# victorramirez952/tomography_3d_reconstructor

Hardware: AMD Instinct MI355X
Metric: Mvoxels/s (SDF+MC) on 1024^3 ellipsoid stack; achieved HBM GB/s vs peak (higher is better)
Workload: dtype f64

## Files before the change

### include/tomo_hip.h

```cpp
#ifndef TOMO_HIP_H
#define TOMO_HIP_H

#include <stddef.h>
#include <stdint.h>

#ifdef __cplusplus
extern "C" {
#endif

#define TOMO_OK 0
#define TOMO_E_ARG (-1)
#define TOMO_E_LAUNCH (-2)
#define TOMO_E_SIZE (-3)
#define TOMO_E_WORKSPACE (-4)

int tomo_abi_version(void);
const char *tomo_error_string(int code);
int tomo_host_mc_cell(const float *h_v, double iso, int8_t *h_tris, int *h_uses_centre);
double tomo_host_mc_edge_offset(double va, double vb);
void tomo_host_mc_centre_offset(const double *h_v8, double *h_out3);

int tomo_host_checksum(const void *h_data, int64_t nbytes, int nthreads, uint64_t *h_out);
int tomo_host_checksum_impl(const void *h_data, int64_t nbytes, int nthreads, int impl, uint64_t *h_out);
int64_t tomo_host_checksum_chunk_bytes(void);
// ... 196 lines not shown
                   const double *xt, double r2, int level, int32_t *map, void *workspace, int64_t workspace_bytes, void *stream);
int tomo_edt_threshold_masked(const uint64_t *sites, int nz, int ny, int nx, const double *zt, const double *yt, const double *xt,
                              int inside, double r2, int keep_less, const uint64_t *mask, uint64_t *out, void *workspace,
                              int64_t workspace_bytes, void *stream);
int tomo_edt_thickness_finish(int32_t *map, const uint64_t *bits, int nz, int ny, int nx, const float *values, int levels,
                              int64_t *counts, void *stream);
int tomo_pack_threshold(const uint8_t *grey, uint64_t *bits, int nz, int ny, int nx, int threshold, void *stream);
int tomo_obj_write(const char *path, const void *vertices, int vertex_is_double, int64_t nv, const int64_t *faces,
                   int64_t nf, int nthreads);
int tomo_obj_block_format(int kind, const void *h_rows, int64_t n, int nthreads, void **h_block, int64_t *h_nbytes);
int tomo_obj_block_pwrite(const char *path, int64_t offset, const void *h_block);
void tomo_obj_block_free(void *h_block);

int tomo_extend_bits(const uint64_t *bits, uint64_t *ext, int nz, int ny, int nx, int pad, void *stream);
int tomo_field_fill(const uint64_t *ext, float *field, int nz, int ny, int nx, int pad, int gaussian,
                    unsigned long long *signs, uint8_t *gcls, void *stream);
int tomo_field_fill_bits(const uint64_t *bits, float *field, int nz, int ny, int nx, int pad, unsigned long long *signs,
                         uint8_t *gcls, void *stream);
int64_t tomo_field_span_bytes(int nz, int ny, int nx, int pad);
int tomo_field_fill_bits_sparse(const uint64_t *bits, float *field, int nz, int ny, int nx, int pad, unsigned long long *signs,
                                uint8_t *gcls, uint8_t *span_ws, void *stream);
int64_t tomo_sign_rows(int Ny);
int64_t tomo_sign_buffer_words(int Nz, int Ny, int Nx, int xorg);
int tomo_field_signs(const float *field, int Nz, int Ny, int Nx, int64_t pitch, int xorg, double iso, int z_begin,
                     int z_end, unsigned long long *signs, uint8_t *gcls, void *stream);

int tomo_mc_classify(const unsigned long long *signs, const uint8_t *gcls, int Nz, int Ny, int Nx, int xorg,
                     unsigned long long *seg_act, uint32_t *seg_cnt, void *stream);
int tomo_mc_scan_segments(const uint32_t *seg_cnt, int64_t nseg, uint32_t *seg_aoff, unsigned long long *totals,
                          void *workspace, int64_t workspace_bytes, void *stream);
int64_t tomo_mc_scan_workspace_bytes(int64_t n);
int tomo_mc_scan(const uint32_t *counts, int64_t n, uint32_t *off_a, uint32_t *off_b,
                 unsigned long long *totals, void *workspace, int64_t workspace_bytes, void *stream);
int tomo_mc_list(int Nz, int Ny, int Nx, int xorg, const uint32_t *seg_aoff, const unsigned long long *seg_act,
                 unsigned long long *vox_key, void *stream);
int tomo_mc_eval(const float *field, int Nz, int Ny, int Nx, int64_t pitch, int xorg, double iso,
                 const unsigned long long *vox_key, int64_t na, uint32_t *vox_counts, uint8_t *vox_flags, void *stream);
int tomo_mc_list_capped(int Nz, int Ny, int Nx, int xorg, const uint32_t *seg_aoff, const unsigned long long *seg_act,
                        unsigned long long *vox_key, int64_t cap, void *stream);
int tomo_mc_eval_capped(const float *field, int Nz, int Ny, int Nx, int64_t pitch, int xorg, double iso,
                        const unsigned long long *vox_key, int64_t cap, const unsigned long long *na_dev,
                        uint32_t *vox_counts, uint8_t *vox_flags, void *stream);
int tomo_mc_emit(const float *field, int Nz, int Ny, int Nx, int64_t pitch, int xorg, double iso,
                 const unsigned long long *vox_key, int64_t na, const unsigned long long *seg_act,
                 const uint32_t *seg_aoff, const uint32_t *vox_voff, const uint32_t *vox_foff, const uint8_t *vox_flags,
                 int z_offset, unsigned long long *vkey, float *vpos, int32_t *faces, unsigned long long *totals,
                 void *stream);

int tomo_mc_first_touch(const float *field, int Nz, int Ny, int Nx, int64_t pitch, int xorg, double iso,
                        const unsigned long long *vox_key, int64_t na, const unsigned long long *seg_act,
                        const uint32_t *seg_aoff, const uint32_t *vox_voff, const uint8_t *vox_flags, int mode,
                        uint32_t *created, const uint32_t *base, int32_t *ft_rank, unsigned long long *totals, void *stream);

int tomo_mc3_list(int Nz, int Ny, int Nx, int xorg, const uint32_t *seg_cnt, const unsigned long long *seg_act,
                  uint32_t *seg_blk, uint32_t *seg_aoff, unsigned long long *vox_key, int64_t cap, unsigned long long *tot,
                  void *stream);
int tomo_mc3_eval(const float *field, int Nz, int Ny, int Nx, int64_t pitch, int xorg, double iso,
                  const unsigned long long *vox_key, int64_t cap, const unsigned long long *tot, int z_offset,
                  uint32_t *vox_loc, int32_t *vox_til, uint8_t *vox_flags, uint16_t *vox_used, float *vox_f3, float *vox_c3,
                  uint32_t *blk3, void *stream);
int64_t tomo_mc3_slice_table_words(int Nz, int Ny);
int64_t tomo_mc3_sort_segments(int Nz, int Ny);
int tomo_mc3_scan(int Nz, int Ny, int Nx, int xorg, const uint32_t *seg_aoff, const uint32_t *vox_loc, int64_t cap,
                  uint32_t *blk3, uint32_t *slice_tab, unsigned long long *tot, int64_t cap_v, int64_t cap_f, void *stream);
int tomo_mc3_vertices(int Nz, int Ny, int Nx, int xorg, const unsigned long long *vox_key, int64_t cap,
                      const unsigned long long *tot, const uint32_t *vox_loc, const uint8_t *vox_flags, const float *vox_f3,
                      const float *vox_c3, const uint32_t *blk3, const uint32_t *slice_tab, int z_offset, int shift,
                      const double *cum, int64_t ncum, const double *adj, int64_t nadj, float mm_y, float mm_x, float *vrec,
                      uint32_t *keys, uint32_t *idx, void *stream);
int64_t tomo_mc3_sort_workspace_bytes(int64_t cap_v, int64_t nseg);
int tomo_mc3_sort_rank_top(const float *vrec, uint32_t *keys, uint32_t *idx, int64_t cap_v, int Nz, int Ny, const uint32_t *slice_tab,
                           unsigned long long *tot, float *uniq, int32_t *table, void *workspace, int64_t workspace_bytes,
                           float z_top, void *stream);
int tomo_mc3_sort_rank_fused(const float *vrec, const uint32_t *keys, int64_t cap_v, int Nz, int Ny, uint32_t *slice_tab,
                             unsigned long long *tot, float *uniq, int32_t *table, float z_top, void *stream);
int tomo_mc3_faces(int Nz, int Ny, int Nx, int xorg, const unsigned long long *vox_key, int64_t cap, unsigned long long *tot,
                   const unsigned long long *seg_act, const uint32_t *seg_aoff, const uint32_t *vox_loc, const int32_t *vox_til,
                   const uint16_t *vox_used, const uint32_t *blk3, const int32_t *table, int64_t *faces, int64_t cap_f,
                   void *stream);

int tomo_vertex_finalize(float *vpos, int64_t nv, int shift, const double *cum, int64_t ncum,
                         const double *adj, int64_t nadj, float mm_y, float mm_x, void *stream);
int64_t tomo_mesh_unique_workspace_bytes(int64_t nv);
int tomo_mesh_unique(const float *vpos, int64_t nv, float *uniq, int32_t *rank, unsigned long long *totals,
                     void *workspace, int64_t workspace_bytes, void *stream);
int tomo_mesh_lookup(const float *uniq, int64_t nu, const float *query, int64_t nq, int32_t *out,
                     unsigned long long *missing, void *stream);
int tomo_slab_top_rows(const float *uniq, const unsigned long long *tot, int64_t cap_v, int64_t cap, float *msg, void *stream);
int tomo_slab_lookup_summary(const float *uniq, const unsigned long long *tot, int64_t cap_v, const float *msg, int64_t cap,
                             int32_t *out, int64_t cap_top, int64_t caller_flags, unsigned long long *scratch, int64_t *summary,
                             void *stream);
int tomo_mc3_faces_slab(int Nz, int Ny, int Nx, int xorg, const unsigned long long *vox_key, int64_t cap, unsigned long long *tot,
                        const unsigned long long *seg_act, const uint32_t *seg_aoff, const uint32_t *vox_loc, const int32_t *vox_til,
                        const uint16_t *vox_used, const uint32_t *blk3, const int32_t *table, int64_t *faces, int64_t cap_f,
                        const int64_t *gathered, int rank, int world, const int32_t *ids_next, int64_t cap_top, int64_t cap_v,
                        void *stream);
int tomo_mesh_volume_area(const float *verts, const int64_t *faces, int64_t nf, double *out, void *stream);

int tomo_layer_colors(const void *verts, int is_f64, int64_t nv, int64_t stride, double start1, double end1, int enable1,
                      double start2, double end2, int enable2, uint8_t *rgba, void *stream);
int64_t tomo_mesh_edge_table_bytes(int64_t nf);
int tomo_mesh_edges(const int64_t *faces, int64_t nf, int64_t nv, void *table, int64_t table_bytes, unsigned long long *counters,
                    void *stream);
int tomo_mesh_seam_edges(const void *table, int64_t table_bytes, int64_t nf, int64_t first_ghost, unsigned long long *msg,
                         int64_t cap, unsigned long long *count, void *stream);
int tomo_mesh_seam_merge(const void *table, int64_t table_bytes, int64_t nf, const unsigned long long *msg, int64_t n,
// ... 21 lines not shown
```

### tomography_3d_reconstructor_amd/_lib.py

```python
import ctypes
import os
import subprocess

_HERE = os.path.dirname(os.path.abspath(__file__))
SO_PATH = os.environ.get("TOMO_LIB") or os.path.join(_HERE, "libtomo_hip.so")
CSRC = os.path.join(_HERE, "csrc")

_c_i = ctypes.c_int
_c_i64 = ctypes.c_int64
_c_p = ctypes.c_void_p
_c_d = ctypes.c_double
_c_f = ctypes.c_float

SIGNATURES = {
    "tomo_abi_version": (_c_i, []),
    "tomo_error_string": (ctypes.c_char_p, [_c_i]),
    "tomo_host_mc_cell": (_c_i, [_c_p, _c_d, _c_p, _c_p]),
    "tomo_host_mc_edge_offset": (_c_d, [_c_d, _c_d]),
    "tomo_host_mc_centre_offset": (None, [_c_p, _c_p]),
    "tomo_host_checksum": (_c_i, [_c_p, _c_i64, _c_i, _c_p]),
    "tomo_host_checksum_impl": (_c_i, [_c_p, _c_i64, _c_i, _c_i, _c_p]),
    "tomo_host_checksum_chunk_bytes": (_c_i64, []),
    "tomo_host_checksum_part": (_c_i, [_c_p, _c_i64, _c_i64, _c_i, _c_i, _c_p]),
    "tomo_host_checksum_fold": (_c_i, [_c_p, _c_i64, _c_i64, _c_p]),
# ... 87 lines not shown
    "tomo_thin_nodes": (_c_i, [_c_p, _c_i, _c_i, _c_i, _c_p, _c_p, _c_p, _c_p]),
    "tomo_thin_count": (_c_i, [_c_p, _c_i, _c_i, _c_i, _c_p, _c_i64, _c_p, _c_p, _c_p, _c_p, _c_p, _c_p, _c_p, _c_i, _c_i, _c_i64, _c_i64,
                               _c_p]),
    "tomo_branch_split": (_c_i, [_c_p, _c_i, _c_i, _c_i, _c_p, _c_p, _c_p, _c_p]),
    "tomo_branch_hist": (_c_i, [_c_p, _c_i, _c_i, _c_i, _c_p, _c_i64, _c_p, _c_p, _c_p, _c_p, _c_i64, _c_p, _c_p, _c_p, _c_i64, _c_p,
                                _c_p]),
    "tomo_branch_attach": (_c_i, [_c_p, _c_i, _c_i, _c_i, _c_p, _c_i64, _c_p, _c_p, _c_p, _c_p, _c_p, _c_p, _c_p, _c_p, _c_i64, _c_i64,
                                  _c_p]),
    "tomo_branch_lookup": (_c_i, [_c_p, _c_i, _c_i, _c_i, _c_p, _c_i64, _c_p, _c_p, _c_p, _c_i64, _c_p, _c_i64, _c_p, _c_p]),
    "tomo_branch_clear": (_c_i, [_c_p, _c_i, _c_i, _c_i, _c_p, _c_i64, _c_p, _c_p, _c_p, _c_p, _c_i64, _c_p, _c_p, _c_p]),
    "tomo_contact_count": (_c_i, [_c_p, _c_p, _c_i, _c_i, _c_i, _c_p, _c_p]),
    "tomo_contact_insert": (_c_i, [_c_p, _c_p, _c_i, _c_i, _c_i, _c_p, _c_p, _c_p, _c_p, _c_i64, _c_p, _c_p, _c_p, _c_p, _c_p, _c_p, _c_p,
                                   _c_p, _c_p]),
    "tomo_contact_hist": (_c_i, [_c_p, _c_p, _c_i, _c_i, _c_i, _c_p, _c_i64, _c_p, _c_p, _c_p, _c_p, _c_p, _c_i64, _c_p, _c_i64, _c_p, _c_p,
                                 _c_p]),
    "tomo_contact_finish": (_c_i, [_c_i64, _c_p, _c_i64, _c_p, _c_p, _c_p, _c_p, _c_p, _c_p, _c_p, _c_p, _c_p, _c_p, _c_i64, _c_p, _c_i, _c_i,
                                   _c_p, _c_p, _c_p]),
    "tomo_pack_threshold": (_c_i, [_c_p, _c_p, _c_i, _c_i, _c_i, _c_i, _c_p]),
    "tomo_obj_write": (_c_i, [ctypes.c_char_p, _c_p, _c_i, _c_i64, _c_p, _c_i64, _c_i]),
    "tomo_obj_block_format": (_c_i, [_c_i, _c_p, _c_i64, _c_i, ctypes.POINTER(_c_p), ctypes.POINTER(_c_i64)]),
    "tomo_obj_block_pwrite": (_c_i, [ctypes.c_char_p, _c_i64, _c_p]),
    "tomo_obj_block_free": (None, [_c_p]),
    "tomo_fill_holes_slice": (_c_i, [_c_p, _c_i, _c_i, _c_i, _c_i, _c_p, _c_p]),
    "tomo_fill_holes_ends": (_c_i, [_c_p, _c_i, _c_i, _c_i, _c_p, _c_p]),
    "tomo_pack_close_ends": (_c_i, [_c_p, _c_p, _c_i, _c_i, _c_i, _c_p, _c_p]),
    "tomo_pack_bits_pair": (_c_i, [_c_p, _c_p, _c_i, _c_p, _c_p, _c_i, _c_i, _c_i, _c_p]),
    "tomo_slab_edges": (_c_i, [_c_p, _c_p, _c_i, _c_i, _c_i, _c_i, _c_p, _c_p, _c_i, _c_i, _c_p, _c_p, _c_p, _c_i, _c_p, _c_p, _c_p, _c_p,
                               _c_i, _c_p, _c_p]),
    "tomo_pack_close_range": (_c_i, [_c_p, _c_p, _c_i, _c_i, _c_i, _c_i, _c_i, _c_p, _c_p, _c_i, _c_i, _c_p]),
    "tomo_close_ends_workspace_words": (_c_i64, [_c_i, _c_i, _c_i]),
    "tomo_close_ends_scan": (_c_i, [_c_p, _c_i, _c_i, _c_i, _c_p, _c_p]),
    "tomo_morph_fused": (_c_i, [_c_p, _c_p, _c_i, _c_i, _c_i, ctypes.c_uint32, _c_i, _c_p]),
    "tomo_smooth": (_c_i, [_c_p, _c_p, _c_i, _c_i, _c_i, _c_i, _c_i, _c_p]),
    "tomo_extend_bits": (_c_i, [_c_p, _c_p, _c_i, _c_i, _c_i, _c_i, _c_p]),
    "tomo_field_fill": (_c_i, [_c_p, _c_p, _c_i, _c_i, _c_i, _c_i, _c_i, _c_p, _c_p, _c_p]),
    "tomo_field_fill_bits": (_c_i, [_c_p, _c_p, _c_i, _c_i, _c_i, _c_i, _c_p, _c_p, _c_p]),
    "tomo_field_span_bytes": (_c_i64, [_c_i, _c_i, _c_i, _c_i]),
    "tomo_field_fill_bits_sparse": (_c_i, [_c_p, _c_p, _c_i, _c_i, _c_i, _c_i, _c_p, _c_p, _c_p, _c_p]),
    "tomo_sign_rows": (_c_i64, [_c_i]),
    "tomo_sign_buffer_words": (_c_i64, [_c_i, _c_i, _c_i, _c_i]),
    "tomo_field_signs": (_c_i, [_c_p, _c_i, _c_i, _c_i, _c_i64, _c_i, _c_d, _c_i, _c_i, _c_p, _c_p, _c_p]),
    "tomo_mc_classify": (_c_i, [_c_p, _c_p, _c_i, _c_i, _c_i, _c_i, _c_p, _c_p, _c_p]),
    "tomo_mc_scan_segments": (_c_i, [_c_p, _c_i64, _c_p, _c_p, _c_p, _c_i64, _c_p]),
    "tomo_mc_scan_workspace_bytes": (_c_i64, [_c_i64]),
    "tomo_mc_scan": (_c_i, [_c_p, _c_i64, _c_p, _c_p, _c_p, _c_p, _c_i64, _c_p]),
    "tomo_mc_list": (_c_i, [_c_i, _c_i, _c_i, _c_i, _c_p, _c_p, _c_p, _c_p]),
    "tomo_mc_eval": (_c_i, [_c_p, _c_i, _c_i, _c_i, _c_i64, _c_i, _c_d, _c_p, _c_i64, _c_p, _c_p, _c_p]),
    "tomo_mc_list_capped": (_c_i, [_c_i, _c_i, _c_i, _c_i, _c_p, _c_p, _c_p, _c_i64, _c_p]),
    "tomo_mc_eval_capped": (_c_i, [_c_p, _c_i, _c_i, _c_i, _c_i64, _c_i, _c_d, _c_p, _c_i64, _c_p, _c_p, _c_p, _c_p]),
    "tomo_mc_emit": (_c_i, [_c_p, _c_i, _c_i, _c_i, _c_i64, _c_i, _c_d, _c_p, _c_i64, _c_p, _c_p, _c_p, _c_p, _c_p, _c_i, _c_p,
                            _c_p, _c_p, _c_p, _c_p]),
    "tomo_mc_first_touch": (_c_i, [_c_p, _c_i, _c_i, _c_i, _c_i64, _c_i, _c_d, _c_p, _c_i64, _c_p, _c_p, _c_p, _c_p, _c_i, _c_p,
                                   _c_p, _c_p, _c_p, _c_p]),
    "tomo_mc3_list": (_c_i, [_c_i, _c_i, _c_i, _c_i, _c_p, _c_p, _c_p, _c_p, _c_p, _c_i64, _c_p, _c_p]),
    "tomo_mc3_eval": (_c_i, [_c_p, _c_i, _c_i, _c_i, _c_i64, _c_i, _c_d, _c_p, _c_i64, _c_p, _c_i, _c_p, _c_p, _c_p, _c_p, _c_p,
                             _c_p, _c_p, _c_p]),
    "tomo_mc3_slice_table_words": (_c_i64, [_c_i, _c_i]),
    "tomo_mc3_sort_segments": (_c_i64, [_c_i, _c_i]),
    "tomo_mc3_scan": (_c_i, [_c_i, _c_i, _c_i, _c_i, _c_p, _c_p, _c_i64, _c_p, _c_p, _c_p, _c_i64, _c_i64, _c_p]),
    "tomo_mc3_vertices": (_c_i, [_c_i, _c_i, _c_i, _c_i, _c_p, _c_i64, _c_p, _c_p, _c_p, _c_p, _c_p, _c_p, _c_p, _c_i, _c_i,
                                 _c_p, _c_i64, _c_p, _c_i64, _c_f, _c_f, _c_p, _c_p, _c_p, _c_p]),
    "tomo_mc3_sort_workspace_bytes": (_c_i64, [_c_i64, _c_i64]),
    "tomo_mc3_sort_rank_top": (_c_i, [_c_p, _c_p, _c_p, _c_i64, _c_i, _c_i, _c_p, _c_p, _c_p, _c_p, _c_p, _c_i64, _c_f, _c_p]),
    "tomo_mc3_sort_rank_fused": (_c_i, [_c_p, _c_p, _c_i64, _c_i, _c_i, _c_p, _c_p, _c_p, _c_p, _c_f, _c_p]),
    "tomo_mc3_faces": (_c_i, [_c_i, _c_i, _c_i, _c_i, _c_p, _c_i64, _c_p, _c_p, _c_p, _c_p, _c_p, _c_p, _c_p, _c_p, _c_p, _c_i64, _c_p]),
    "tomo_vertex_finalize": (_c_i, [_c_p, _c_i64, _c_i, _c_p, _c_i64, _c_p, _c_i64, _c_f, _c_f, _c_p]),
    "tomo_mesh_unique_workspace_bytes": (_c_i64, [_c_i64]),
    "tomo_mesh_unique": (_c_i, [_c_p, _c_i64, _c_p, _c_p, _c_p, _c_p, _c_i64, _c_p]),
    "tomo_mesh_lookup": (_c_i, [_c_p, _c_i64, _c_p, _c_i64, _c_p, _c_p, _c_p]),
    "tomo_slab_top_rows": (_c_i, [_c_p, _c_p, _c_i64, _c_i64, _c_p, _c_p]),
    "tomo_slab_lookup_summary": (_c_i, [_c_p, _c_p, _c_i64, _c_p, _c_i64, _c_p, _c_i64, _c_i64, _c_p, _c_p, _c_p]),
    "tomo_mc3_faces_slab": (_c_i, [_c_i, _c_i, _c_i, _c_i, _c_p, _c_i64, _c_p, _c_p, _c_p, _c_p, _c_p, _c_p, _c_p, _c_p, _c_p, _c_i64,
                                   _c_p, _c_i, _c_i, _c_p, _c_i64, _c_i64, _c_p]),
    "tomo_mesh_volume_area": (_c_i, [_c_p, _c_p, _c_i64, _c_p, _c_p]),
    "tomo_layer_colors": (_c_i, [_c_p, _c_i, _c_i64, _c_i64, _c_d, _c_d, _c_i, _c_d, _c_d, _c_i, _c_p, _c_p]),
    "tomo_mesh_edge_table_bytes": (_c_i64, [_c_i64]),
    "tomo_mesh_edges": (_c_i, [_c_p, _c_i64, _c_i64, _c_p, _c_i64, _c_p, _c_p]),
    "tomo_mesh_seam_edges": (_c_i, [_c_p, _c_i64, _c_i64, _c_i64, _c_p, _c_i64, _c_p, _c_p]),
    "tomo_mesh_seam_merge": (_c_i, [_c_p, _c_i64, _c_i64, _c_p, _c_i64, _c_p, _c_p]),
    "tomo_mesh_orient_workspace_bytes": (_c_i64, [_c_i64]),
    "tomo_mesh_orient": (_c_i, [_c_p, _c_i64, _c_i64, _c_p, _c_i64, _c_p, _c_p, _c_p]),
    "tomo_mesh_signed_volume": (_c_i, [_c_p, _c_p, _c_i64, _c_p, _c_p, _c_p]),
    "tomo_glb_pack_faces": (_c_i, [_c_p, _c_i64, _c_p, _c_p, _c_p, _c_i, _c_p]),
    "tomo_glb_pack_positions": (_c_i, [_c_p, _c_i, _c_i64, _c_p, _c_p, _c_p]),
    "tomo_mesh_vertex_normals_workspace_bytes": (_c_i64, [_c_i64, _c_i64]),
    "tomo_mesh_vertex_normals": (_c_i, [_c_p, _c_i64, _c_p, _c_i, _c_i64, _c_p, _c_i64, _c_p, _c_p, _c_p]),
    "tomo_mesh_vertex_normals_seeded": (_c_i, [_c_p, _c_i64, _c_p, _c_i, _c_i64, _c_p, _c_i64, _c_p, _c_p, _c_p, _c_i64, _c_p, _c_i64,
                                              _c_i, _c_p]),
}

_LIB = None


class TomoError(RuntimeError):
    pass


class TomoUnavailable(TomoError):
    """No MI355X visible / libtomo_hip.so not built.  The one failure the drop-in classes never turn into the
    reference's `return None`: there is no CPU fallback to hide behind."""


def build(force=False):
    srcs = [os.path.join(CSRC, f) for f in os.listdir(CSRC) if f.endswith((".hip", ".h", ".cpp", "Makefile"))]
    srcs.append(os.path.join(_HERE, "..", "include", "tomo_hip.h"))
    stale = force or not os.path.exists(SO_PATH) or any(
# ... 28 lines not shown
```

### tomography_3d_reconstructor_amd/csrc/mc.hip

```cpp
#include <cstring>
#include <cstdlib>
#include "tomo_common.h"
#include <rocprim/rocprim.hpp>

#define MC_LUT_QUAL __device__ const
#define MC_FN __device__ static inline
#include "mc_cell.h"

#define SEG 256
#define KEY_XBITS 20
static_assert(KEY_XBITS + 2 == TOMO_KEY_ROW_SHIFT, "key layout shared with mesh.hip");

struct McGrid {
    int Nz, Ny, Nx;
    int64_t pitch;
    int xorg;
    int segs_per_row;
    double iso;
};

typedef float float4u __attribute__((ext_vector_type(4), aligned(4)));
typedef float float2u __attribute__((ext_vector_type(2), aligned(4)));
typedef float float3u __attribute__((ext_vector_type(3), aligned(4)));
typedef int int3u __attribute__((ext_vector_type(3), aligned(4)));
// ... 654 lines not shown
        const int64_t rowY = (int64_t)g.Ny;
        for (int k = 0; k < 3 * t.ntri; k++) {
            int ed = t.tris[k];
            if (seen & (1u << ed)) continue;
            seen |= 1u << ed;
            const int dx = (mc_edges_displaced(0) >> ed) & 1, dy = (mc_edges_displaced(1) >> ed) & 1;
            const int dz = (mc_edges_displaced(2) >> ed) & 1;
            const int slot = ((mc_edges_slot_bit(0) >> ed) & 1) | ((mc_edges_slot_bit(1) >> ed) & 1) << 1;
            int ox = c.X + dx, oy = c.Y + dy, oz = c.Z + dz;
            bool creator;
            if (slot == 0) creator = (dy == (oy > 0 ? 1 : 0)) && (dz == (oz > 0 ? 1 : 0));
            else if (slot == 1) creator = (dx == (ox > 0 ? 1 : 0)) && (dz == (oz > 0 ? 1 : 0));
            else if (slot == 2) creator = (dx == (ox > 0 ? 1 : 0)) && (dy == (oy > 0 ? 1 : 0));
            else creator = true;
            if (!creator) continue;
            if (mode == 1) {
                u32 v;
                if ((dx | dy | dz) == 0) v = slot_vertex(vox_voff[i], (u32)flags, slot);
                else v = find_vertex(make_key(c.row + dy + dz * rowY, ox, 0), slot, g, seg_act, seg_aoff, vox_voff, vox_flags);
                if (v == 0xffffffffu) atomicAdd(&totals[3], 1ull);
                else ft_rank[v] = (int32_t)(base[i] + n);
            }
            n++;
        }
    }
    if (mode == 0) created[i] = n;
}

TOMO_API int tomo_mc_first_touch(const float *field, int Nz, int Ny, int Nx, int64_t pitch, int xorg, double iso,
                                 const unsigned long long *vox_key, int64_t na, const unsigned long long *seg_act,
                                 const uint32_t *seg_aoff, const uint32_t *vox_voff, const uint8_t *vox_flags, int mode,
                                 uint32_t *created,
                                 const uint32_t *base, int32_t *ft_rank, unsigned long long *totals, void *stream)
{
    McGrid g;
    if (const int rc = make_grid(g, field, Nz, Ny, Nx, pitch, xorg, iso)) return rc;
    if (!vox_key || !seg_act || !seg_aoff || !vox_voff || !vox_flags || !totals || (mode == 0 && !created) ||
        (mode == 1 && (!base || !ft_rank)) || (mode != 0 && mode != 1))
        return TOMO_E_ARG;
    if (na <= 0) return TOMO_OK;
    int64_t blocks = ceil_div64(na, 256);
    if (blocks > 0x7fffffff) return TOMO_E_SIZE;
    hipLaunchKernelGGL(mc_first_touch_kernel, dim3((unsigned)blocks), dim3(256), 0, (hipStream_t)stream, field, g,
                       (const u64 *)vox_key, na, (const u64 *)seg_act, seg_aoff, vox_voff, vox_flags, mode, created, base, ft_rank,
                       (u64 *)totals);
    return tomo_status();
}

#define MC3_BLK 256
#define MC3_LOC_A(l) ((l) & 1023u)
#define MC3_LOC_B(l) (((l) >> 10) & 1023u)
#define MC3_LOC_T(l) ((l) >> 20)

__global__ __launch_bounds__(256) void mc3_segsum_kernel(const u32 *__restrict__ seg_cnt, int64_t nseg, u32 *__restrict__ seg_blk,
                                                         int64_t nblk)
{
    const int lane = threadIdx.x & 63;
    const int64_t b = (int64_t)blockIdx.x * 4 + (threadIdx.x >> 6);
    if (b >= nblk) return;
    const int64_t i0 = b * MC3_BLK + lane * 4;
    u32 s = 0;
    if (i0 + 3 < nseg) {
        const uint4 v = *(const uint4 *)(seg_cnt + i0);
        s = v.x + v.y + v.z + v.w;
    } else {
        for (int k = 0; k < 4; k++) if (i0 + k < nseg) s += seg_cnt[i0 + k];
    }
    s = wave_sum(s);
    if (lane == 0) seg_blk[b] = s;
}

template <int K>
__device__ static inline void scan_small_inplace(u32 *__restrict__ a, int64_t stride, int64_t n, u64 *total_out, u32 *lds )
{
    const int lane = threadIdx.x & 63, w = threadIdx.x >> 6;
    u32 carry[K];
    u64 wide[K];
#pragma unroll
    for (int k = 0; k < K; k++) { carry[k] = 0; wide[k] = 0; }
    for (int64_t base = 0; base < n; base += 1024 * 8) {
        const int64_t i0 = base + (int64_t)threadIdx.x * 8;
        u32 v[K][8], s[K];
#pragma unroll
        for (int k = 0; k < K; k++) {
            u32 *p = a + k * stride + i0;
            if (i0 + 7 < n && ((uintptr_t)p & 15) == 0) {
                const uint4 lo = *(const uint4 *)p, hi = *(const uint4 *)(p + 4);
                v[k][0] = lo.x; v[k][1] = lo.y; v[k][2] = lo.z; v[k][3] = lo.w; v[k][4] = hi.x; v[k][5] = hi.y; v[k][6] = hi.z; v[k][7] = hi.w;
            } else {
#pragma unroll
                for (int j = 0; j < 8; j++) v[k][j] = i0 + j < n ? p[j] : 0u;
            }
            s[k] = 0;
#pragma unroll
            for (int j = 0; j < 8; j++) s[k] += v[k][j];
        }
        u32 inc[K];
#pragma unroll
        for (int k = 0; k < K; k++) {
            inc[k] = wave_inclusive_scan(s[k]);
            if (lane == 63) lds[k * 16 + w] = inc[k];
        }
        __syncthreads();
        if (w == 0) {
#pragma unroll
            for (int k = 0; k < K; k++) {
                const u32 t = lane < 16 ? lds[k * 16 + lane] : 0u;
                const u32 ti = wave_inclusive_scan(t);
                if (lane < 16) lds[k * 16 + lane] = ti - t;
                if (lane == 15) lds[K * 16 + k] = ti;
            }
        }
        __syncthreads();
#pragma unroll
        for (int k = 0; k < K; k++) {
            u32 ex = carry[k] + lds[k * 16 + w] + inc[k] - s[k];
            u32 *p = a + k * stride + i0;
            if (i0 + 7 < n && ((uintptr_t)p & 15) == 0) {
                uint4 lo, hi;
                lo.x = ex; ex += v[k][0]; lo.y = ex; ex += v[k][1]; lo.z = ex; ex += v[k][2]; lo.w = ex; ex += v[k][3];
                hi.x = ex; ex += v[k][4]; hi.y = ex; ex += v[k][5]; hi.z = ex; ex += v[k][6]; hi.w = ex;
                *(uint4 *)p = lo; *(uint4 *)(p + 4) = hi;
            } else {
#pragma unroll
                for (int j = 0; j < 8; j++) { if (i0 + j < n) p[j] = ex; ex += v[k][j]; }
            }
            carry[k] += lds[K * 16 + k];
            wide[k] += lds[K * 16 + k];
        }
        __syncthreads();
    }
#pragma unroll
    for (int k = 0; k < K; k++) total_out[k] = wide[k];
}

__global__ __launch_bounds__(1024) void mc3_scan_seg_kernel(u32 *__restrict__ seg_blk, int64_t nblk, u64 *__restrict__ tot)
{
    __shared__ u32 lds[17];
    u64 total;
    scan_small_inplace<1>(seg_blk, 0, nblk, &total, lds);
    if (threadIdx.x == 0) {
        tot[0] = total;
        tot[1] = tot[2] = tot[4] = tot[5] = tot[6] = tot[7] = 0ull;
        tot[3] = total > 0xffffffffull ? 1ull : 0ull;
    }
}

__global__ __launch_bounds__(MC3_BLK) void mc3_list_kernel(const McGrid g, const u32 *__restrict__ seg_cnt,
                                                           const u32 *__restrict__ seg_blk, const u64 *__restrict__ seg_act,
                                                           int64_t nseg, u32 *__restrict__ seg_aoff, u64 *__restrict__ vox_key,
                                                           u32 cap, u64 *__restrict__ tot)
{
    __shared__ u32 wsum[4];
    const int lane = threadIdx.x & 63, w = threadIdx.x >> 6;
    const int64_t seg = (int64_t)blockIdx.x * MC3_BLK + threadIdx.x;
    const u32 cnt = seg < nseg ? seg_cnt[seg] : 0u;
    const u32 inc = wave_inclusive_scan(cnt);
    if (lane == 63) wsum[w] = inc;
    __syncthreads();
    u32 o = seg_blk[blockIdx.x] + inc - cnt;
    for (int k = 0; k < w; k++) o += wsum[k];
    if (seg >= nseg) return;
    seg_aoff[seg] = o;
    if (seg == nseg - 1) seg_aoff[nseg] = o + cnt;
    if (cnt == 0) return;
    if ((u64)o + cnt > (u64)cap || tot[0] > (u64)cap) {
        if (o <= cap) atomicOr((unsigned long long *)&tot[3], 1ull);
        return;
    }
    seg_write_keys(g, seg, seg_act, o, vox_key);
}

TOMO_API int tomo_mc3_list(int Nz, int Ny, int Nx, int xorg, const uint32_t *seg_cnt, const unsigned long long *seg_act,
                           uint32_t *seg_blk, uint32_t *seg_aoff, unsigned long long *vox_key, int64_t cap,
                           unsigned long long *tot, void *stream)
{
    if (!seg_cnt || !seg_act || !seg_blk || !seg_aoff || !vox_key || !tot) return TOMO_E_ARG;
    McGrid g;
    if (const int rc = index_grid(g, Nz, Ny, Nx, xorg)) return rc;
    if (cap <= 0 || cap >= 0x1fffffffll) return TOMO_E_SIZE;
    const int64_t nseg = (int64_t)Nz * Ny * g.segs_per_row, nblk = ceil_div64(nseg, MC3_BLK);
    if (nblk > 0x7fffffff) return TOMO_E_SIZE;
    hipStream_t s = (hipStream_t)stream;
    hipLaunchKernelGGL(mc3_segsum_kernel, dim3((unsigned)ceil_div64(nblk, 4)), dim3(256), 0, s, seg_cnt, nseg, seg_blk, nblk);
    hipLaunchKernelGGL(mc3_scan_seg_kernel, dim3(1), dim3(1024), 0, s, seg_blk, nblk, (u64 *)tot);
    hipLaunchKernelGGL(mc3_list_kernel, dim3((unsigned)nblk), dim3(MC3_BLK), 0, s, g, seg_cnt, (const u32 *)seg_blk,
                       (const u64 *)seg_act, nseg, seg_aoff, (u64 *)vox_key, (u32)cap, (u64 *)tot);
    return tomo_status();
}

__global__ __launch_bounds__(MC3_BLK) void mc3_eval_kernel(const float *__restrict__ field, const McGrid g,
                                                           const u64 *__restrict__ vox_key, int64_t cap,
                                                           const u64 *__restrict__ tot, int z_offset,
                                                           u32 *__restrict__ vox_loc, int32_t *__restrict__ vox_til,
                                                           uint8_t *__restrict__ vox_flags, uint16_t *__restrict__ vox_used,
                                                           float *__restrict__ vox_f3, float *__restrict__ vox_c3,
                                                           u32 *__restrict__ blk3, int64_t nblk)
{
    __shared__ u32 wsum[4];
    const int lane = threadIdx.x & 63, w = threadIdx.x >> 6;
    const int64_t i = (int64_t)blockIdx.x * MC3_BLK + threadIdx.x;
    const u64 na = tot[0];
    const bool live = i < cap && (u64)i < na && na <= (u64)cap;
    u32 packed = 0;
    if (live) {
        Cell c;
        load_cell(field, g, vox_key[i], c);
        int ntri = 0;
        int32_t til = 0;
        u32 used = 0;
        if (c.cell_ok && c.index != 0 && c.index != 255) {
            const McTiling t = mc_cell_tiling(c.v, c.index);
            ntri = t.ntri;
            if (t.centre) c.flags |= 8;
            til = (int32_t)(((intptr_t)t.tris - (intptr_t)LUT_TILING1) * 16 + ntri);
            used = mc_used_edges(c.index) | (t.centre ? 1u << 12 : 0u);
            if (ntri == 0) used = 0;
        }
        const int Zg = c.Z + z_offset;
        float3u f3;
        f3.x = (float)((double)Zg + mc_edge_offset(c.v[0], c.v[4]));
        f3.y = (float)((double)c.Y + mc_edge_offset(c.v[0], c.v[3]));
        f3.z = (float)((double)c.X + mc_edge_offset(c.v[0], c.v[1]));
        *(float3u *)(vox_f3 + 3 * i) = f3;
        if (c.flags & 8) {
            double ox, oy, oz;
            mc_centre_offset(c.v, &ox, &oy, &oz);
            *(float3u *)(vox_c3 + 3 * i) = (float3u){(float)((double)Zg + oz), (float)((double)c.Y + oy), (float)((double)c.X + ox)};
        }
        vox_til[i] = til;
        vox_flags[i] = (uint8_t)c.flags;
        vox_used[i] = (uint16_t)used;
        packed = (u32)__popc(c.flags & 3) | ((u32)__popc(c.flags & 12) << 10) | ((u32)ntri << 20);
    }
    const u32 inc = wave_inclusive_scan(packed);
    if (lane == 63) wsum[w] = inc;
    __syncthreads();
    u32 ex = inc - packed;
    for (int k = 0; k < w; k++) ex += wsum[k];
// ... 326 lines not shown
```

### tomography_3d_reconstructor_amd/pipeline.py

```python
import math
import os
import threading
from dataclasses import dataclass

import numpy as np
import torch

from . import _lib


COUNTERS = dict.fromkeys(("na_hint_hit", "na_hint_miss", "mc3_hint_hit", "mc3_hint_miss", "mc3_sort_fused", "mc3_sort_library",
                          "mc3_exact", "mc3_general_unique", "mc3_degenerate", "components_label", "components_expand",
                          "components_filter", "slab_components_label", "slab_components_seam", "slab_components_merge",
                          "slab_components_expand", "slab_components_filter", "distance_transform", "distance_offset",
                          "components_measure", "components_zhist", "components_moments", "components_euler",
                          "components_cavities", "local_thickness", "opening_volume", "components_surface", "components_fill",
                          "components_cavity_owners", "component_thickness", "components_value", "components_levels", "component_caliper",
                          "geodesic_calls", "geodesic_sweeps", "component_geodesic", "zone_calls", "zone_sweeps", "zone_cuts",
                          "separate_components", "zone_contacts", "contact_launches", "recon_calls", "recon_sweeps",
                          "thin_calls", "thin_iterations", "thin_passes", "thin_nodes", "component_skeleton",
                          "skeleton_branches", "branch_split", "skeleton_branches_hist", "branch_attach", "branch_lookup", "branch_clear",
                          "prune_rounds"), 0)
NA_HINTS = os.environ.get("TOMO_NA_HINTS", "1") not in ("", "0")
_NA_HINT = {}
# ... 2723 lines not shown
            raise _lib.TomoError("%s did not arrive within %.0f s: the GPU is stuck or a neighbour rank has left the job" % (what, timeout_s))
        if dt > 2e-3:
            time.sleep(1e-4)


class PendingDownload:
    _free = {}

    def __init__(self, t):
        t = t.reshape(-1)
        self._key = (str(t.device), threading.get_ident(), int(t.numel()))
        pool = PendingDownload._free.setdefault(self._key, [])
        self._host = pool.pop() if pool else torch.empty(t.numel(), dtype=torch.int64, pin_memory=True)
        self._host.copy_(t, non_blocking=True)
        self._event = torch.cuda.Event()
        self._event.record(torch.cuda.current_stream(t.device))

    def wait(self, timeout_s=None):
        if timeout_s is None:
            self._event.synchronize()
        else:
            wait_event(self._event, timeout_s, "the counters of a pass")
        out = self._host.tolist()
        PendingDownload._free[self._key].append(self._host)
        self._host = None
        return out


class Mc3Surface:

    def __init__(self, f, slice_depths, mm_per_pixel_y, mm_per_pixel_x, add_padding=True, z_offset=0, z_top=None, tot=None):
        self.field, self.z_offset = f, int(z_offset)
        self.z_top = float("nan") if z_top is None else float(z_top)
        self.hint_key = (f.Nz, f.Ny, f.Nx, self.z_offset)
        self._depth = _depth_args(slice_depths, add_padding, f.data.device)
        self._mm = (float(np.float32(mm_per_pixel_y)), float(np.float32(mm_per_pixel_x)))
        self.tot = torch.empty(8, dtype=torch.int64, device=f.data.device) if tot is None else tot
        self.uniq = self.table = self.faces_final = None
        self.nv = self.nf = self.na = 0
        self.deferred = False
        self._pending = None

    def classify(self):
        L, f, dev = _lib.lib(), self.field, self.field.data.device
        if f.signs is None or f.signs_level != 0.5:
            if f.sparse:
                raise _lib.TomoError("a sparse field holds floats only near the 0.5 surface")
            field_signs(f, 0.5)
        nseg = f.Nz * f.Ny * L.tomo_mc_segments_per_row(f.Nx, f.xorg)
        self.seg_act = torch.empty(nseg * 4, dtype=torch.int64, device=dev)
        self.seg_cnt = torch.empty(nseg, dtype=torch.int32, device=dev)
        _lib.check(L.tomo_mc_classify(_p(f.signs), _p(f.gcls), f.Nz, f.Ny, f.Nx, f.xorg, _p(self.seg_act), _p(self.seg_cnt), _stream()),
                   "tomo_mc_classify")
        self.seg_blk = torch.empty((nseg + 255) // 256, dtype=torch.int32, device=dev)
        self.seg_aoff = torch.empty(nseg + 1, dtype=torch.int32, device=dev)

    def build_list(self, cap):
        f, self.cap = self.field, cap
        self.vox_key = torch.empty(cap, dtype=torch.int64, device=f.data.device)
        _lib.check(_lib.lib().tomo_mc3_list(f.Nz, f.Ny, f.Nx, f.xorg, _p(self.seg_cnt), _p(self.seg_act), _p(self.seg_blk), _p(self.seg_aoff),
                                            _p(self.vox_key), cap, _p(self.tot), _stream()), "tomo_mc3_list")

    def eval_scan(self, cap_v, cap_f):
        L, f, cap, st, dev = _lib.lib(), self.field, self.cap, _stream(), self.field.data.device
        self.vox_loc = torch.empty(cap, dtype=torch.int32, device=dev)
        self.vox_til = torch.empty(cap, dtype=torch.int32, device=dev)
        self.vox_flags = torch.empty(cap, dtype=torch.uint8, device=dev)
        self.vox_used = torch.empty(cap, dtype=torch.int16, device=dev)
        self.vox_f3 = torch.empty(3 * cap, dtype=torch.float32, device=dev)
        self.vox_c3 = torch.empty(3 * cap, dtype=torch.float32, device=dev)
        self.blk3 = torch.empty(3 * ((cap + 255) // 256), dtype=torch.int32, device=dev)
        self.slice_tab = torch.empty(L.tomo_mc3_slice_table_words(f.Nz, f.Ny), dtype=torch.int32, device=dev)
        _lib.check(L.tomo_mc3_eval(_p(f.data), f.Nz, f.Ny, f.Nx, f.pitch, f.xorg, 0.5, _p(self.vox_key), cap, _p(self.tot), self.z_offset,
                                   _p(self.vox_loc), _p(self.vox_til), _p(self.vox_flags), _p(self.vox_used), _p(self.vox_f3),
                                   _p(self.vox_c3), _p(self.blk3), st), "tomo_mc3_eval")
        _lib.check(L.tomo_mc3_scan(f.Nz, f.Ny, f.Nx, f.xorg, _p(self.seg_aoff), _p(self.vox_loc), cap, _p(self.blk3), _p(self.slice_tab),
                                   _p(self.tot), cap_v, cap_f, st), "tomo_mc3_scan")

    def vertices_sort(self, cap_v):
        L, f, cap, tot, st, dev = _lib.lib(), self.field, self.cap, self.tot, _stream(), self.field.data.device
        cum_t, ncum, adj_t, nadj = self._depth
        self.cap_v = cap_v
        self.vrec = torch.empty((cap_v, 4), dtype=torch.float32, device=dev)
        keys = torch.empty(cap_v, dtype=torch.int32, device=dev)
        self.rows = torch.empty((cap_v, 3), dtype=torch.float32, device=dev)
        self.table = torch.empty(4 * cap, dtype=torch.int32, device=dev)
        fused = FUSED_SORT and not _MC3_LARGE.get(self.hint_key)
        idx = None if fused else torch.empty(cap_v, dtype=torch.int32, device=dev)
        _lib.check(L.tomo_mc3_vertices(f.Nz, f.Ny, f.Nx, f.xorg, _p(self.vox_key), cap, _p(tot), _p(self.vox_loc), _p(self.vox_flags),
                                       _p(self.vox_f3), _p(self.vox_c3), _p(self.blk3), _p(self.slice_tab), self.z_offset, 1, _p(cum_t), ncum,
                                       _p(adj_t), nadj, *self._mm, _p(self.vrec), _p(keys), _p(idx), st), "tomo_mc3_vertices")
        if fused:
            COUNTERS["mc3_sort_fused"] += 1
            _lib.check(L.tomo_mc3_sort_rank_fused(_p(self.vrec), _p(keys), cap_v, f.Nz, f.Ny, _p(self.slice_tab), _p(tot), _p(self.rows),
                                                  _p(self.table), self.z_top, st), "tomo_mc3_sort_rank_fused")
            return
        COUNTERS["mc3_sort_library"] += 1
        wsb = L.tomo_mc3_sort_workspace_bytes(cap_v, L.tomo_mc3_sort_segments(f.Nz, f.Ny))
        ws = torch.empty(wsb, dtype=torch.uint8, device=dev)
        _lib.check(L.tomo_mc3_sort_rank_top(_p(self.vrec), _p(keys), _p(idx), cap_v, f.Nz, f.Ny, _p(self.slice_tab), _p(tot), _p(self.rows),
                                            _p(self.table), _p(ws), wsb, self.z_top, st), "tomo_mc3_sort_rank_top")

    def enqueue(self, cap, cap_v, cap_f):
        self.build_list(cap)
        self.eval_scan(cap_v, cap_f)
        self.vertices_sort(cap_v)
        self.cap_f = cap_f

    def faces(self, table=None, again=False, slab_map=None):
        L = _lib.lib()
        f, st = self.field, _stream()
        tab = self.table if table is None else table
# ... 408 lines not shown
```

Measured before the change: 679,600.

## Fold single-block segment scan into segsum and list kernels via grouped carries

Removes the single-workgroup mc3_scan_seg_kernel launch. The segsum kernel now has each workgroup scan a contiguous group of up to 256 group-blocks, writing in-group prefix sums plus one group total. The list kernel rebuilds its global offset from the previous block's prefix plus a wave reduction over the group totals. This cuts a serial one-block kernel and a launch from the list stage, at the cost of a larger seg_blk buffer and a redundant group-total reduction in every list block.

```diff
diff --git a/include/tomo_hip.h b/include/tomo_hip.h
--- a/include/tomo_hip.h
+++ b/include/tomo_hip.h
@@ -272,6 +272,7 @@
                         const uint32_t *seg_aoff, const uint32_t *vox_voff, const uint8_t *vox_flags, int mode,
                         uint32_t *created, const uint32_t *base, int32_t *ft_rank, unsigned long long *totals, void *stream);
 
+int64_t tomo_mc3_list_blk_words(int64_t nseg);
 int tomo_mc3_list(int Nz, int Ny, int Nx, int xorg, const uint32_t *seg_cnt, const unsigned long long *seg_act,
                   uint32_t *seg_blk, uint32_t *seg_aoff, unsigned long long *vox_key, int64_t cap, unsigned long long *tot,
                   void *stream);
diff --git a/tomography_3d_reconstructor_amd/_lib.py b/tomography_3d_reconstructor_amd/_lib.py
--- a/tomography_3d_reconstructor_amd/_lib.py
+++ b/tomography_3d_reconstructor_amd/_lib.py
@@ -163,6 +163,7 @@
                             _c_p, _c_p, _c_p, _c_p]),
     "tomo_mc_first_touch": (_c_i, [_c_p, _c_i, _c_i, _c_i, _c_i64, _c_i, _c_d, _c_p, _c_i64, _c_p, _c_p, _c_p, _c_p, _c_i, _c_p,
                                    _c_p, _c_p, _c_p, _c_p]),
+    "tomo_mc3_list_blk_words": (_c_i64, [_c_i64]),
     "tomo_mc3_list": (_c_i, [_c_i, _c_i, _c_i, _c_i, _c_p, _c_p, _c_p, _c_p, _c_p, _c_i64, _c_p, _c_p]),
     "tomo_mc3_eval": (_c_i, [_c_p, _c_i, _c_i, _c_i, _c_i64, _c_i, _c_d, _c_p, _c_i64, _c_p, _c_i, _c_p, _c_p, _c_p, _c_p, _c_p,
                              _c_p, _c_p, _c_p]),
diff --git a/tomography_3d_reconstructor_amd/csrc/mc.hip b/tomography_3d_reconstructor_amd/csrc/mc.hip
--- a/tomography_3d_reconstructor_amd/csrc/mc.hip
+++ b/tomography_3d_reconstructor_amd/csrc/mc.hip
@@ -730,22 +730,74 @@
 #define MC3_LOC_B(l) (((l) >> 10) & 1023u)
 #define MC3_LOC_T(l) ((l) >> 20)
 
+#define MC3_GRP_ROUND 64
+#define MC3_GRP_LIMIT 256
+#define MC3_GRP_MAX_SHIFT 15
+
+static int mc3_group_shift(int64_t nblk)
+{
+    int sh = 6;
+    static_assert(MC3_GRP_ROUND == 1 << 6, "a group is a whole number of rounds");
+    while (sh < MC3_GRP_MAX_SHIFT && ceil_div64(nblk, (int64_t)1 << sh) > MC3_GRP_LIMIT) sh++;
+    return sh;
+}
+
+TOMO_API int64_t tomo_mc3_list_blk_words(int64_t nseg)
+{
+    if (nseg <= 0) return 0;
+    const int64_t nblk = ceil_div64(nseg, 256);
+    return nblk + ceil_div64(nblk, (int64_t)1 << mc3_group_shift(nblk));
+}
+
 __global__ __launch_bounds__(256) void mc3_segsum_kernel(const u32 *__restrict__ seg_cnt, int64_t nseg, u32 *__restrict__ seg_blk,
-                                                         int64_t nblk)
-{
-    const int lane = threadIdx.x & 63;
-    const int64_t b = (int64_t)blockIdx.x * 4 + (threadIdx.x >> 6);
-    if (b >= nblk) return;
-    const int64_t i0 = b * MC3_BLK + lane * 4;
-    u32 s = 0;
-    if (i0 + 3 < nseg) {
-        const uint4 v = *(const uint4 *)(seg_cnt + i0);
-        s = v.x + v.y + v.z + v.w;
-    } else {
-        for (int k = 0; k < 4; k++) if (i0 + k < nseg) s += seg_cnt[i0 + k];
-    }
-    s = wave_sum(s);
-    if (lane == 0) seg_blk[b] = s;
+                                                         int64_t nblk, int gshift, u64 *__restrict__ tot)
+{
+    __shared__ u32 wtot[4];
+    const int lane = threadIdx.x & 63, w = threadIdx.x >> 6;
+    const int64_t b0 = (int64_t)blockIdx.x << gshift;
+    const int rounds = 1 << (gshift - 6);
+    u32 carry = 0;
+    for (int r = 0; r < rounds; r++) {
+        if (b0 + (int64_t)r * MC3_GRP_ROUND >= nblk) break;
+        const int64_t bw = b0 + (int64_t)r * MC3_GRP_ROUND + w * 16;
+        u32 s[16];
+        if ((bw + 16) * MC3_BLK <= nseg) {
+            uint4 v[16];
+#pragma unroll
+            for (int j = 0; j < 16; j++) v[j] = *(const uint4 *)(seg_cnt + (bw + j) * MC3_BLK + lane * 4);
+#pragma unroll
+            for (int j = 0; j < 16; j++) s[j] = v[j].x + v[j].y + v[j].z + v[j].w;
+        } else {
+#pragma unroll
+            for (int j = 0; j < 16; j++) {
+                const int64_t i0 = (bw + j) * MC3_BLK + lane * 4;
+                s[j] = 0;
+                for (int k = 0; k < 4; k++) if (i0 + k < nseg) s[j] += seg_cnt[i0 + k];
+            }
+        }
+        u32 mine = 0;
+#pragma unroll
+        for (int j = 0; j < 16; j++) {
+            const u32 t = wave_sum(s[j]);
+            if (lane == j) mine = t;
+        }
+        const u32 inc = wave_inclusive_scan(mine);
+        if (lane == 63) wtot[w] = inc;
+        __syncthreads();
+        u32 pre = carry, all = 0;
+#pragma unroll
+        for (int k = 0; k < 4; k++) {
+            if (k < w) pre += wtot[k];
+            all += wtot[k];
+        }
+        if (lane < 16 && bw + lane < nblk) seg_blk[bw + lane] = pre + inc;
+        carry += all;
+        __syncthreads();
+    }
+    if (threadIdx.x == 0) {
+        seg_blk[nblk + blockIdx.x] = carry;
+        if (blockIdx.x == 0) tot[1] = tot[2] = tot[3] = tot[4] = tot[5] = tot[6] = tot[7] = 0ull;
+    }
 }
 
 template <int K>
@@ -812,37 +864,46 @@
     for (int k = 0; k < K; k++) total_out[k] = wide[k];
 }
 
-__global__ __launch_bounds__(1024) void mc3_scan_seg_kernel(u32 *__restrict__ seg_blk, int64_t nblk, u64 *__restrict__ tot)
-{
-    __shared__ u32 lds[17];
-    u64 total;
-    scan_small_inplace<1>(seg_blk, 0, nblk, &total, lds);
-    if (threadIdx.x == 0) {
-        tot[0] = total;
-        tot[1] = tot[2] = tot[4] = tot[5] = tot[6] = tot[7] = 0ull;
-        tot[3] = total > 0xffffffffull ? 1ull : 0ull;
-    }
-}
-
 __global__ __launch_bounds__(MC3_BLK) void mc3_list_kernel(const McGrid g, const u32 *__restrict__ seg_cnt,
-                                                           const u32 *__restrict__ seg_blk, const u64 *__restrict__ seg_act,
-                                                           int64_t nseg, u32 *__restrict__ seg_aoff, u64 *__restrict__ vox_key,
-                                                           u32 cap, u64 *__restrict__ tot)
-{
-    __shared__ u32 wsum[4];
+                                                           const u32 *__restrict__ seg_blk, int64_t nblk, int gshift,
+                                                           const u64 *__restrict__ seg_act, int64_t nseg,
+                                                           u32 *__restrict__ seg_aoff, u64 *__restrict__ vox_key, u32 cap,
+                                                           u64 *__restrict__ tot)
+{
+    __shared__ u32 wsum[4], s_base;
+    __shared__ u64 s_all;
     const int lane = threadIdx.x & 63, w = threadIdx.x >> 6;
-    const int64_t seg = (int64_t)blockIdx.x * MC3_BLK + threadIdx.x;
+    const int64_t blk = blockIdx.x, seg = blk * MC3_BLK + threadIdx.x;
     const u32 cnt = seg < nseg ? seg_cnt[seg] : 0u;
+    const u32 prev = (blk & (((int64_t)1 << gshift) - 1)) ? seg_blk[blk - 1] : 0u;
+    if (w == 0) {
+        const int64_t grp = blk >> gshift, ngrp = ((nblk - 1) >> gshift) + 1;
+        u32 base = 0;
+        u64 all = 0;
+        for (int64_t t = lane; t < ngrp; t += 64) {
+            const u32 v = seg_blk[nblk + t];
+            all += v;
+            if (t < grp) base += v;
+        }
+        base = wave_sum(base);
+        all = wave_sum64(all);
+        if (lane == 0) { s_base = base; s_all = all; }
+    }
     const u32 inc = wave_inclusive_scan(cnt);
     if (lane == 63) wsum[w] = inc;
     __syncthreads();
-    u32 o = seg_blk[blockIdx.x] + inc - cnt;
+    u32 o = prev + s_base + inc - cnt;
     for (int k = 0; k < w; k++) o += wsum[k];
+    const u64 all = s_all;
+    if (blk == 0 && threadIdx.x == 0) {
+        tot[0] = all;
+        if (all > 0xffffffffull) atomicOr((unsigned long long *)&tot[3], 1ull);
+    }
     if (seg >= nseg) return;
     seg_aoff[seg] = o;
     if (seg == nseg - 1) seg_aoff[nseg] = o + cnt;
     if (cnt == 0) return;
-    if ((u64)o + cnt > (u64)cap || tot[0] > (u64)cap) {
+    if ((u64)o + cnt > (u64)cap || all > (u64)cap) {
         if (o <= cap) atomicOr((unsigned long long *)&tot[3], 1ull);
         return;
     }
@@ -859,10 +920,11 @@
     if (cap <= 0 || cap >= 0x1fffffffll) return TOMO_E_SIZE;
     const int64_t nseg = (int64_t)Nz * Ny * g.segs_per_row, nblk = ceil_div64(nseg, MC3_BLK);
     if (nblk > 0x7fffffff) return TOMO_E_SIZE;
+    const int gshift = mc3_group_shift(nblk);
     hipStream_t s = (hipStream_t)stream;
-    hipLaunchKernelGGL(mc3_segsum_kernel, dim3((unsigned)ceil_div64(nblk, 4)), dim3(256), 0, s, seg_cnt, nseg, seg_blk, nblk);
-    hipLaunchKernelGGL(mc3_scan_seg_kernel, dim3(1), dim3(1024), 0, s, seg_blk, nblk, (u64 *)tot);
-    hipLaunchKernelGGL(mc3_list_kernel, dim3((unsigned)nblk), dim3(MC3_BLK), 0, s, g, seg_cnt, (const u32 *)seg_blk,
+    hipLaunchKernelGGL(mc3_segsum_kernel, dim3((unsigned)ceil_div64(nblk, (int64_t)1 << gshift)), dim3(256), 0, s, seg_cnt, nseg,
+                       seg_blk, nblk, gshift, (u64 *)tot);
+    hipLaunchKernelGGL(mc3_list_kernel, dim3((unsigned)nblk), dim3(MC3_BLK), 0, s, g, seg_cnt, (const u32 *)seg_blk, nblk, gshift,
                        (const u64 *)seg_act, nseg, seg_aoff, (u64 *)vox_key, (u32)cap, (u64 *)tot);
     return tomo_status();
 }
diff --git a/tomography_3d_reconstructor_amd/pipeline.py b/tomography_3d_reconstructor_amd/pipeline.py
--- a/tomography_3d_reconstructor_amd/pipeline.py
+++ b/tomography_3d_reconstructor_amd/pipeline.py
@@ -2799,12 +2799,14 @@
         self.seg_cnt = torch.empty(nseg, dtype=torch.int32, device=dev)
         _lib.check(L.tomo_mc_classify(_p(f.signs), _p(f.gcls), f.Nz, f.Ny, f.Nx, f.xorg, _p(self.seg_act), _p(self.seg_cnt), _stream()),
                    "tomo_mc_classify")
-        self.seg_blk = torch.empty((nseg + 255) // 256, dtype=torch.int32, device=dev)
+        self.seg_blk = torch.empty(L.tomo_mc3_list_blk_words(nseg), dtype=torch.int32, device=dev)
         self.seg_aoff = torch.empty(nseg + 1, dtype=torch.int32, device=dev)
 
     def build_list(self, cap):
         f, self.cap = self.field, cap
         self.vox_key = torch.empty(cap, dtype=torch.int64, device=f.data.device)
+        if self.seg_blk.numel() < _lib.lib().tomo_mc3_list_blk_words(self.seg_cnt.numel()):
+            raise ValueError("seg_blk is shorter than tomo_mc3_list_blk_words(nseg)")
         _lib.check(_lib.lib().tomo_mc3_list(f.Nz, f.Ny, f.Nx, f.xorg, _p(self.seg_cnt), _p(self.seg_act), _p(self.seg_blk), _p(self.seg_aoff),
                                             _p(self.vox_key), cap, _p(self.tot), _stream()), "tomo_mc3_list")
 
```

Result: no change. 680,300, median of 6 (+0.1%).
